# lh3/miniasm

Hardware: NVIDIA H100
Metric: paf_overlaps_per_sec_ingest_to_gfa (higher is better)
Workload: dtype int64/uint32 (+3 float32 predicates)

## Files before the change

### miniasm_b200/csrc/ingest_dev.cu

```cuda
#include "ingest_dev.cuh"
#include "shard_comm.cuh"
#include <cub/cub.cuh>

struct PLine {
	uint32_t ql, qs, qe, tl, ts, te, ml_rev, bl;
	uint32_t tdelta;
	uint32_t qnl, tnl;
	uint32_t nf;
};

struct __align__(16) PRec {
	uint32_t qs, qe, ts, te;
	uint32_t ml_rev;
	uint32_t bl_f;
	uint32_t slot_q, slot_t;
};
static_assert(sizeof(PRec) == 32, "PRec layout");
constexpr uint32_t NOSLOT = 0xffffffffu;

constexpr int NL_THREADS = 256;
constexpr int NL_PER_THREAD = 4;
constexpr uint64_t NL_TILE = (uint64_t)NL_THREADS * NL_PER_THREAD * 16;

__device__ __forceinline__ uint32_t nl_mask4(uint32_t w) { return __vcmpeq4(w, 0x0a0a0a0au); }
// ... 103 lines not shown
#ifdef __CUDA_ARCH__
				const int pos = off + __ffs(bits) - 1;
#else
				const int pos = off + __builtin_ctz(bits);
#endif
				bits &= bits - 1;
				if (pos >= 0 && pos < (int)len && nt < 11) tab[nt++ * 32] = (uint32_t)pos;
			}
		}
	}
	const uint32_t nf = nt + 1 < 11 ? nt + 1 : 11;
	#define COL_S(k) ((k) ? tab[((k) - 1) * 32] + 1 : 0u)
	#define COL_T(k) ((uint32_t)(k) < nt ? tab[(k) * 32] : len)
	memset(&r, 0, sizeof(r));
	r.nf = nf;
	r.qnl = COL_T(0);
	if (nf > 1) r.ql = num_field(p, COL_S(1), COL_T(1));
	if (nf > 2) r.qs = num_field(p, COL_S(2), COL_T(2));
	if (nf > 3) r.qe = num_field(p, COL_S(3), COL_T(3));
	if (nf > 4) { const uint32_t s4 = COL_S(4); r.ml_rev = (COL_T(4) > s4 && p[s4] == '-') ? 0x80000000u : 0; }
	if (nf > 5) {
		const uint32_t s5 = COL_S(5), t5 = COL_T(5);
		r.tnl = t5 - s5, r.tdelta = s5;
	}
	if (nf > 6) r.tl = num_field(p, COL_S(6), COL_T(6));
	if (nf > 7) r.ts = num_field(p, COL_S(7), COL_T(7));
	if (nf > 8) r.te = num_field(p, COL_S(8), COL_T(8));
	if (nf > 9) r.ml_rev |= num_field(p, COL_S(9), COL_T(9)) & 0x7fffffffu;
	if (nf > 10) r.bl = num_field(p, COL_S(10), COL_T(10));
	#undef COL_S
	#undef COL_T
}

struct NameTab {
	unsigned long long *key;
	unsigned long long *first;
	uint32_t *id;
	uint64_t mask;
	uint32_t *hits = nullptr;
};
constexpr int NT_OFF_BITS = 37;
constexpr unsigned long long NT_OFF_MASK = (1ull << NT_OFF_BITS) - 1;

__device__ __forceinline__ uint32_t tab_insert(const NameTab &t, const char *__restrict__ text, const char *nm, uint32_t nl, uint64_t goff, uint64_t occ,
                                               unsigned long long *overflow)
{
	const uint64_t h = name_hash(nm, 0, nl, 0);
	const unsigned long long mine = (h >> 37) << NT_OFF_BITS | (goff + 1);
	uint64_t s = h & t.mask;
	for (int probe = 0; probe < 1 << 14; ++probe, s = (s + 1) & t.mask) {
		unsigned long long k = t.key[s];
		if (k == 0) {
			k = atomicCAS(&t.key[s], 0ull, mine);
			if (k == 0) k = mine;
		}
		if ((k ^ mine) >> NT_OFF_BITS) continue;
		bool same = k == mine;
		if (!same) {
			const char *w = text + ((k & NT_OFF_MASK) - 1);
			same = true;
			for (uint32_t i = 0; same && i < nl; ++i) same = w[i] == nm[i];
			same = same && w[nl] == '\t';
		}
		if (!same) continue;
		if (t.first[s] > occ) atomicMin(&t.first[s], (unsigned long long)occ);
		return (uint32_t)s;
	}
	atomicAdd(overflow, 1ull);
	return 0;
}

constexpr int PT_THREADS = 128;
constexpr uint32_t PT_TILE = 8192;
constexpr uint32_t PT_OVER = 1024;
constexpr uint32_t PT_LIST = 1024;
static_assert(PT_TILE == PT_THREADS * 64, "each thread scans 64 bytes of its tile for line starts");
static_assert(PT_OVER % 16 == 0 && PT_OVER <= PT_TILE, "the overhang ends inside the tile after the parsed ones");

typedef cub::ScanTileState<unsigned long long> LineTileState;
typedef cub::TilePrefixCallbackOp<unsigned long long, ::cuda::std::plus<unsigned long long>, LineTileState> LinePrefixOp;

enum { PC_PARSED = 0, PC_STORED, PC_OVERFLOW, PC_LINES, PC_CUT, PC_N };

__device__ __forceinline__ uint32_t nl_bits_u4(const uint4 w)
{
	const uint32_t m[4] = { nl_mask4(w.x), nl_mask4(w.y), nl_mask4(w.z), nl_mask4(w.w) };
	uint32_t bits = 0;
	#pragma unroll
	for (int k = 0; k < 4; ++k) bits |= ((m[k] & 1) | (m[k] >> 7 & 2) | (m[k] >> 14 & 4) | (m[k] >> 21 & 8)) << (4 * k);
	return bits;
}

__global__ void k_tiles_init(LineTileState ts, int n_tile) { ts.InitializeStatus(n_tile); }

__global__ void __launch_bounds__(PT_THREADS)
k_parse_tiles(const char *__restrict__ text, size_t len, size_t avail, uint64_t t_lo, unsigned *tile_ctr, LineTileState tstate,
              int min_span, int min_match, int bi_dir, NameTab tab, PRec *out, uint64_t *start, uint64_t line_cap, unsigned long long *counts)
{
	typedef cub::BlockScan<uint32_t, PT_THREADS> BS;
	__shared__ __align__(16) char s_text[PT_TILE + PT_OVER + 16];
	__shared__ uint16_t s_start[PT_LIST + 1];
	__shared__ uint32_t s_vals[PT_THREADS / 32][11][32];
// ... 52 lines not shown
				if (e == ~0ull) atomicAdd(counts + PC_CUT, 1ull);
			}
		}
		__syncthreads();
		last_eol = s_eol;
	}
	unsigned n_parsed = 0, n_pass = 0;
	for (uint32_t r0 = 0; r0 < n; r0 += PT_LIST) {
		{
			uint32_t r = rank;
			uint64_t b = bits;
			if (line0) { if (r == r0) s_start[0] = 0; ++r; }
			for (; b && r <= r0 + PT_LIST; ++r, b &= b - 1)
				if (r >= r0) s_start[r - r0] = (uint16_t)(my0 + __ffsll((long long)b));
		}
		__syncthreads();
		const uint32_t cnt = n - r0 < PT_LIST ? n - r0 : PT_LIST;
		for (uint32_t j0 = 0; j0 < cnt; j0 += PT_THREADS) {
			const uint32_t j = j0 + threadIdx.x;
			const uint64_t i = first + r0 + j;
			uint32_t sq = NOSLOT, st = 0;
			if (j < cnt && i < line_cap) {
				const uint64_t s = b0 + s_start[j];
				uint64_t eol = r0 + j + 1 < n ? b0 + s_start[j + 1] - 1 : last_eol;
				if (eol != ~0ull) {
					const char *base = eol <= w_end ? s_text - b0 : text;
					if (eol - s > 1 && base[eol - 1] == '\r') --eol;
					PLine r;
					parse_line(base + s, base + eol, r, &s_vals[threadIdx.x >> 5][0][lane]);
					if (r.nf >= 10) {
						++n_parsed;
						if (!(r.qe - r.qs < (uint32_t)min_span || r.te - r.ts < (uint32_t)min_span || (int)(r.ml_rev & 0x7fffffffu) < min_match)) {
							++n_pass;
							sq = tab_insert(tab, text, base + s, r.qnl, s, 2 * i, counts + PC_OVERFLOW);
							st = tab_insert(tab, text, base + s + r.tdelta, r.tnl, s + r.tdelta, 2 * i + 1, counts + PC_OVERFLOW);
						}
					}
					start[i] = s;
					*reinterpret_cast<uint4*>(out + i) = make_uint4(r.qs, r.qe, r.ts, r.te);
					*(reinterpret_cast<uint4*>(out + i) + 1) = make_uint4(r.ml_rev, (r.bl & 0x7fffffffu) | (r.nf >= 11 ? 0x80000000u : 0u), sq, st);
				}
			}
			if (tab.hits) {
				const unsigned grp = __match_any_sync(0xffffffffu, sq);
				if (sq != NOSLOT && lane == (uint32_t)__ffs(grp) - 1) atomicAdd(&tab.hits[sq], (uint32_t)__popc(grp));
				if (sq != NOSLOT && bi_dir && st != sq) atomicAdd(&tab.hits[st], 1u);
			}
		}
		__syncthreads();
	}
	n_parsed = __reduce_add_sync(0xffffffffu, n_parsed), n_pass = __reduce_add_sync(0xffffffffu, n_pass);
	if (lane == 0) {
		if (n_parsed) atomicAdd(counts + PC_PARSED, (unsigned long long)n_parsed);
		if (n_pass) atomicAdd(counts + PC_STORED, (unsigned long long)n_pass);
	}
}

__device__ __forceinline__ uint32_t line_bl(const PRec *ln, uint64_t i, uint32_t carry_bl)
{
	if (ln[i].bl_f >> 31) return ln[i].bl_f & 0x7fffffffu;
	for (uint64_t j = i; j-- > 0;)
		if (ln[j].bl_f >> 31) return ln[j].bl_f & 0x7fffffffu;
	return carry_bl & 0x7fffffffu;
}

struct SlotUsed {
	const unsigned long long *first;
	__device__ __forceinline__ bool operator()(uint64_t s) const { return first[s] != ~0ull; }
};

__device__ __forceinline__ void occ_name(const char *text, const uint64_t *start, uint64_t occ, uint64_t *noff, uint32_t *nlen, uint32_t *slen)
{
	const char *p = text + start[occ >> 1];
	uint64_t q = 0;
	if (occ & 1) { int tabs = 0; while (tabs < 5) tabs += p[q++] == '\t'; }
	uint64_t e = q;
	while (p[e] != '\t') ++e;
	*noff = start[occ >> 1] + q, *nlen = (uint32_t)(e - q);
	uint64_t f = e + 1;
	while (p[f] != '\t') ++f;
	*slen = field_to_u32(p + e + 1, p + f);
}

__global__ void k_nocont_mark(const PRec *ln, uint64_t n_lines, const char *text, const uint64_t *start, int max_hang, float int_frac, uint8_t *excl)
{
	for (uint64_t i = blockIdx.x * (uint64_t)blockDim.x + threadIdx.x; i < n_lines; i += (uint64_t)gridDim.x * blockDim.x) {
		const PRec r = ln[i];
		if (r.slot_q == NOSLOT) continue;
		uint64_t no; uint32_t nl, ql, tl;
		occ_name(text, start, 2 * i, &no, &nl, &ql);
		occ_name(text, start, 2 * i + 1, &no, &nl, &tl);
		const bool rev = r.ml_rev >> 31;
		const int l5 = (int)(rev ? tl - r.te : r.ts), l3 = (int)(rev ? r.ts : tl - r.te);
		if (ql >> 1 > tl) {
			if (l5 > max_hang >> 2 || l3 > max_hang >> 2 || (float)(r.te - r.ts) < __fmul_rn((float)tl, int_frac)) continue;
			if ((int)r.qs - l5 > max_hang << 1 && (int)(ql - r.qe) - l3 > max_hang << 1) excl[r.slot_t] = 1;
		} else if (ql < tl >> 1) {
			if (r.qs > (uint32_t)(max_hang >> 2) || ql - r.qe > (uint32_t)(max_hang >> 2) || (float)(r.qe - r.qs) < __fmul_rn((float)ql, int_frac)) continue;
			if (l5 - (int)r.qs > max_hang << 1 && l3 - (int)(ql - r.qe) > max_hang << 1) excl[r.slot_q] = 1;
		}
	}
}

__global__ void k_nocont_drop(PRec *ln, uint64_t n_lines, const uint8_t *excl, int bi_dir, NameTab t)
{
	for (uint64_t i = blockIdx.x * (uint64_t)blockDim.x + threadIdx.x; i < n_lines; i += (uint64_t)gridDim.x * blockDim.x) {
		const uint32_t sq = ln[i].slot_q, st = ln[i].slot_t;
		if (sq == NOSLOT) continue;
		if (excl[sq] || excl[st]) { ln[i].slot_q = NOSLOT; continue; }
		if (t.first[sq] > 2 * i) atomicMin(&t.first[sq], (unsigned long long)(2 * i));
		if (t.first[st] > 2 * i + 1) atomicMin(&t.first[st], (unsigned long long)(2 * i + 1));
		atomicAdd(&t.hits[sq], 1u);
		if (bi_dir && st != sq) atomicAdd(&t.hits[st], 1u);
	}
}

__global__ void k_count_u8(const uint8_t *a, uint64_t n, unsigned long long *out)
{
	unsigned c = 0;
	for (uint64_t i = blockIdx.x * (uint64_t)blockDim.x + threadIdx.x; i < n; i += (uint64_t)gridDim.x * blockDim.x) c += a[i] != 0;
	c = __reduce_add_sync(0xffffffffu, c);
	if ((threadIdx.x & 31) == 0 && c) atomicAdd(out, (unsigned long long)c);
}

__global__ void k_dict_pairs(const uint64_t *slots, uint32_t n, NameTab t, unsigned long long *first_out)
{
	for (uint32_t i = blockIdx.x * blockDim.x + threadIdx.x; i < n; i += gridDim.x * blockDim.x) first_out[i] = t.first[slots[i]];
}

__global__ void k_dict_rank(const unsigned long long *first_sorted, const uint64_t *slot_sorted, uint32_t n, NameTab t,
                            const char *text, const uint64_t *start, uint64_t *noff, uint32_t *nlen, uint32_t *slen, unsigned long long *tot_len,
                            uint32_t *read_cnt)
{
	unsigned long long sum = 0;
	for (uint32_t i = blockIdx.x * blockDim.x + threadIdx.x; i < n; i += gridDim.x * blockDim.x) {
		t.id[slot_sorted[i]] = i;
		read_cnt[i] = t.hits[slot_sorted[i]];
		occ_name(text, start, first_sorted[i], &noff[i], &nlen[i], &slen[i]);
		sum += slen[i];
	}
	typedef cub::BlockReduce<unsigned long long, 256> BR;
	__shared__ typename BR::TempStorage ts;
	unsigned long long s = BR(ts).Sum(sum);
	if (threadIdx.x == 0 && s) atomicAdd(tot_len, s);
}

__global__ void k_hit_emit(const PRec *ln, uint64_t n_lines, int bi_dir, NameTab t, const uint32_t *__restrict__ first, uint32_t *cur, DHit *out)
{
	for (uint64_t i = blockIdx.x * (uint64_t)blockDim.x + threadIdx.x; i < n_lines; i += (uint64_t)gridDim.x * blockDim.x) {
		const PRec r = ln[i];
		if (r.slot_q == NOSLOT) continue;
		const uint32_t qid = t.id[r.slot_q], tid = t.id[r.slot_t], bl = line_bl(ln, i, 0), ord = (uint32_t)(2 * i);
		uint4 *o = reinterpret_cast<uint4*>(out + first[qid] + atomicAdd(&cur[qid], 1u));
		o[0] = make_uint4(r.qs, ord, r.qe, tid);
		o[1] = make_uint4(r.ts, r.te, r.ml_rev, bl);
		if (bi_dir && qid != tid) {
			o = reinterpret_cast<uint4*>(out + first[tid] + atomicAdd(&cur[tid], 1u));
			o[0] = make_uint4(r.ts, ord + 1, r.te, qid);
			o[1] = make_uint4(r.qs, r.qe, r.ml_rev, bl);
		}
// ... 1 lines not shown
}

uint64_t *dev_line_starts(MabDev &d, const char *d_text, size_t len, uint64_t *n_lines_out)
{
	const uint64_t n_tile = (len + NL_TILE - 1) / NL_TILE;
	uint64_t *cnt = mab_alloc<uint64_t>(d, n_tile + 1);
	uint64_t *base = mab_alloc<uint64_t>(d, n_tile + 1);
	MAB_LAUNCH(d, k_nl_count, mab_grid(n_tile, 1, MAB_SMS * 32u), NL_THREADS, 0, d_text, len, n_tile, cnt);
	size_t tb = 0;
	cub::DeviceScan::ExclusiveSum(nullptr, tb, cnt, base, (int64_t)(n_tile + 1), d.stream);
	void *tmp = d.tmp(tb);
	cub::DeviceScan::ExclusiveSum(tmp, tb, cnt, base, (int64_t)(n_tile + 1), d.stream);
	++d.n_lib;
	uint64_t n_nl;
	MAB_CUDA(cudaMemcpyAsync(&n_nl, base + n_tile, 8, cudaMemcpyDeviceToHost, d.stream));
	d.sync();
	const uint64_t n_lines = n_nl + 1;
	uint64_t *start = mab_alloc<uint64_t>(d, n_lines + 1);
	MAB_CUDA(cudaMemsetAsync(start, 0, 8, d.stream));
	MAB_LAUNCH(d, k_nl_write, mab_grid(n_tile, 1, MAB_SMS * 32u), NL_THREADS, 0, d_text, len, n_tile, base, start + 1);
	d.free(cnt); d.free(base);
	*n_lines_out = n_lines;
	return start;
}

void names_free(MabDev &d, DNames &n)
{
	d.free(n.off); d.free(n.nlen); d.free(n.slen);
	n = DNames();
}

static inline uint32_t bits_for(uint64_t x) { uint32_t b = 0; while (x) ++b, x >>= 1; return b ? b : 1; }

static NameTab tab_alloc(MabDev &d, uint64_t cap, bool with_hits)
{
	NameTab tab;
	tab.key = (unsigned long long*)mab_alloc<uint64_t>(d, cap);
	tab.first = (unsigned long long*)mab_alloc<uint64_t>(d, cap);
	tab.id = mab_alloc<uint32_t>(d, cap);
	tab.mask = cap - 1;
	MAB_CUDA(cudaMemsetAsync(tab.key, 0, cap * 8, d.stream));
	MAB_CUDA(cudaMemsetAsync(tab.first, 0xff, cap * 8, d.stream));
	if (with_hits) {
		tab.hits = mab_alloc<uint32_t>(d, cap);
		MAB_CUDA(cudaMemsetAsync(tab.hits, 0, cap * 4, d.stream));
	}
	return tab;
}

static void tab_free(MabDev &d, NameTab &t)
{
	d.free(t.key); d.free(t.first); d.free(t.id);
	if (t.hits) d.free(t.hits);
	t = NameTab{nullptr, nullptr, nullptr, 0};
}

struct Parsed {
	uint64_t *start = nullptr;
	PRec *ln = nullptr;
	NameTab tab{nullptr, nullptr, nullptr, 0};
	uint64_t cap = 0, n_lines = 0, n_parsed = 0;
};

static inline uint64_t line_estimate(size_t len) { return len / 24 + 1024; }
static inline uint64_t tab_cap_for(uint64_t line_cap) { uint64_t cap = 1ull << 20; while (cap < line_cap / 8) cap <<= 1; return cap; }

static LineTileState tiles_alloc(MabDev &d, uint64_t n_tile, void **mem)
{
	if (n_tile >= (1ull << 31) - 64) { fprintf(stderr, "[E::miniasm_b200] more than 2^31 tiles of PAF on one GPU\n"); exit(73); }
	size_t bytes = 0;
	MAB_CUDA(LineTileState::AllocationSize((int)n_tile, bytes));
	*mem = d.alloc(bytes);
	LineTileState ts;
	MAB_CUDA(ts.Init((int)n_tile, *mem, bytes));
	return ts;
}

static void tiles_reset(MabDev &d, LineTileState ts, uint64_t n_tile)
{
	MAB_LAUNCH(d, k_tiles_init, mab_grid(n_tile, 256, 1u << 30), 256, 0, ts, (int)n_tile);
}

static void parse_resident(MabDev &d, const char *d_text, size_t len, int min_span, int min_match, int bi_dir, bool count_hits, Parsed &p)
{
	const uint64_t n_tile = (len + PT_TILE - 1) / PT_TILE;
	uint64_t line_cap = line_estimate(len), cap = tab_cap_for(line_cap);
	unsigned *ctr = mab_alloc<unsigned>(d, 1);
	void *ts_mem = nullptr;
	const LineTileState ts = tiles_alloc(d, n_tile, &ts_mem);
	for (;;) {
		p.start = mab_alloc<uint64_t>(d, line_cap);
		p.ln = mab_alloc<PRec>(d, line_cap);
		p.tab = tab_alloc(d, cap, count_hits);
// ... 83 lines not shown
	p.cap = cap;
	return true;
}

void ingest_paf_stream(MabDev &d, char *d_text, const char *host_text, size_t len, int min_span, int min_match, int bi_dir,
                       DHits &h, DNames &names, IngestStats &st)
{
	memset(&st, 0, sizeof(st));
	names = DNames();
	h.n = 0, h.n_seq = 0;
	if (len == 0) { dh_reserve(d, h, 1); return; }
	if (len >= (1ull << NT_OFF_BITS) - 1) { fprintf(stderr, "[E::miniasm_b200] more than 2^37 bytes of PAF on one GPU\n"); exit(73); }
	Parsed p;
	if (!stream_parse(d, d_text, host_text, len, min_span, min_match, bi_dir, true, p)) {
		ingest_paf(d, d_text, len, min_span, min_match, bi_dir, h, names, st, nullptr);
		return;
	}
	st.n_parsed = p.n_parsed, st.n_lines = p.n_lines;
	d.trace("ingest:stream (copy + parse + dictionary + hit counts)");
	ingest_finish(d, d_text, len, p.start, p.ln, p.n_lines, p.tab, p.cap, bi_dir, nullptr, h, names, st);
}

static void ingest_finish(MabDev &d, const char *d_text, size_t len, uint64_t *start, PRec *ln, uint64_t n_lines, NameTab tab, uint64_t cap, int bi_dir,
                          const NoContParams *nocont, DHits &h, DNames &names, IngestStats &st)
{
	if (2 * n_lines >= (1ull << 32)) { fprintf(stderr, "[E::miniasm_b200] more than 2^31 PAF lines on one GPU\n"); exit(73); }
	d.trace("ingest:dictionary");
	if (nocont) {
		uint8_t *excl = mab_alloc<uint8_t>(d, cap);
		MAB_CUDA(cudaMemsetAsync(excl, 0, cap, d.stream));
		MAB_LAUNCH(d, k_nocont_mark, mab_grid(n_lines, 256), 256, 0, ln, n_lines, d_text, start, nocont->max_hang, nocont->int_frac, excl);
		d.zero_scal(SC_AUX, 1);
		MAB_LAUNCH(d, k_count_u8, mab_grid(cap, 256), 256, 0, excl, cap, d.d_scal + SC_AUX);
		MAB_CUDA(cudaMemsetAsync(tab.first, 0xff, cap * 8, d.stream));
		MAB_CUDA(cudaMemsetAsync(tab.hits, 0, cap * 4, d.stream));
		MAB_LAUNCH(d, k_nocont_drop, mab_grid(n_lines, 256), 256, 0, ln, n_lines, excl, bi_dir, tab);
		st.n_dropped = d.get_scal(SC_AUX);
		d.free(excl);
		d.trace("ingest:-R prefilter");
	}
	uint64_t *slots = mab_alloc<uint64_t>(d, cap);
	uint32_t n_seq;
	{
		cub::CountingInputIterator<uint64_t> pos(0);
		SlotUsed used{tab.first};
		size_t tb = 0;
		unsigned long long *d_n = d.d_scal + SC_NSEL;
		cub::DeviceSelect::If(nullptr, tb, pos, slots, d_n, (int64_t)cap, used, d.stream);
		void *tmp = d.tmp(tb);
		cub::DeviceSelect::If(tmp, tb, pos, slots, d_n, (int64_t)cap, used, d.stream);
		++d.n_lib;
		uint64_t n = d.get_scal(SC_NSEL);
		if (n >= (1ull << 31)) { fprintf(stderr, "[E::miniasm_b200] more than 2^31 reads\n"); exit(73); }
		n_seq = (uint32_t)n;
	}
	names.n_seq = n_seq;
	names.off = mab_alloc<uint64_t>(d, n_seq); names.nlen = mab_alloc<uint32_t>(d, n_seq); names.slen = mab_alloc<uint32_t>(d, n_seq);
	uint32_t *read_cnt = mab_alloc<uint32_t>(d, (size_t)n_seq + 1), *first = mab_alloc<uint32_t>(d, (size_t)n_seq + 1);
	MAB_CUDA(cudaMemsetAsync(read_cnt + n_seq, 0, 4, d.stream));
	if (n_seq) {
		unsigned long long *fa = (unsigned long long*)mab_alloc<uint64_t>(d, n_seq), *fb = (unsigned long long*)mab_alloc<uint64_t>(d, n_seq);
		uint64_t *sb = mab_alloc<uint64_t>(d, n_seq);
		MAB_LAUNCH(d, k_dict_pairs, mab_grid(n_seq, 256), 256, 0, slots, n_seq, tab, fa);
		cub::DoubleBuffer<unsigned long long> dk(fa, fb);
		cub::DoubleBuffer<uint64_t> dv(slots, sb);
		size_t tb = 0;
		int end_bit = (int)bits_for(2 * n_lines + 1);
		cub::DeviceRadixSort::SortPairs(nullptr, tb, dk, dv, (int)n_seq, 0, end_bit, d.stream);
		void *tmp = d.tmp(tb);
		cub::DeviceRadixSort::SortPairs(tmp, tb, dk, dv, (int)n_seq, 0, end_bit, d.stream);
		++d.n_lib;
		d.zero_scal(SC_AUX, 1);
		MAB_LAUNCH(d, k_dict_rank, mab_grid(n_seq, 256), 256, 0, dk.Current(), dv.Current(), n_seq, tab, d_text, start, names.off, names.nlen, names.slen, d.d_scal + SC_AUX,
		           read_cnt);
		st.tot_len = d.get_scal(SC_AUX);
		d.free(fa); d.free(fb); d.free(sb);
	}
	d.free(slots);
// ... 15 lines not shown
	dh_sort_buckets(d, h, first);
	d.free(read_cnt); d.free(first);
	d.trace("ingest:sort_hits");
}

extern "C" int mab_test_parse_line(const char *line, size_t len, uint32_t *out)
{
	static uint32_t vals[11 * 32];
	PLine r;
	size_t eol = len;
	if (eol > 1 && line[eol - 1] == '\r') --eol;
	parse_line(line, line + eol, r, vals);
	out[0] = r.nf, out[1] = r.ql, out[2] = r.qs, out[3] = r.qe, out[4] = r.ml_rev >> 31, out[5] = r.tl, out[6] = r.ts, out[7] = r.te;
	out[8] = r.ml_rev & 0x7fffffffu, out[9] = r.bl, out[10] = r.qnl, out[11] = r.tnl, out[12] = r.tdelta;
	return 0;
}

__global__ void k_last_bl(const PRec *ln, uint64_t n_lines, unsigned long long *out)
{
	unsigned long long mx = 0;
	for (uint64_t i = blockIdx.x * (uint64_t)blockDim.x + threadIdx.x; i < n_lines; i += (uint64_t)gridDim.x * blockDim.x)
		if (ln[i].bl_f >> 31) mx = i + 1;
	#pragma unroll
	for (int o = 16; o; o >>= 1) { unsigned long long t = __shfl_xor_sync(0xffffffffu, mx, o); mx = t > mx ? t : mx; }
	if ((threadIdx.x & 31) == 0 && mx) atomicMax(out, mx);
}

struct GEntry { unsigned long long hash, first; uint32_t slen, nlen; };

__global__ void k_local_entries(const uint64_t *slots, uint32_t n, NameTab t, const char *text, const uint64_t *start, uint64_t line_base, uint64_t seed,
                                GEntry *ent, uint32_t *name_sz, uint64_t *name_off)
{
	for (uint32_t i = blockIdx.x * blockDim.x + threadIdx.x; i < n; i += gridDim.x * blockDim.x) {
		const uint64_t occ = t.first[slots[i]];
		GEntry e;
		uint64_t no;
		occ_name(text, start, occ, &no, &e.nlen, &e.slen);
		e.hash = name_hash(text + no, 0, e.nlen, seed), e.first = 2 * line_base + occ;
		ent[i] = e;
		name_sz[i] = e.nlen, name_off[i] = no;
	}
}

__global__ void k_local_names(uint32_t n, const uint64_t *name_off, const uint32_t *name_sz, const char *text, const uint64_t *pos, char *out)
{
	for (uint32_t i = blockIdx.x * blockDim.x + threadIdx.x; i < n; i += gridDim.x * blockDim.x) {
		const char *src = text + name_off[i];
		char *dst = out + pos[i];
		for (uint32_t k = 0; k < name_sz[i]; ++k) dst[k] = src[k];
	}
}

struct U32ToU64i { __host__ __device__ __forceinline__ uint64_t operator()(uint32_t x) const { return x; } };

struct GTab { unsigned long long *key, *first; uint32_t *win, *id; uint64_t mask; };

__global__ void k_gtab_insert(const GEntry *ent, uint64_t n, GTab t, uint32_t *slot_of, unsigned long long *overflow)
{
	for (uint64_t i = blockIdx.x * (uint64_t)blockDim.x + threadIdx.x; i < n; i += (uint64_t)gridDim.x * blockDim.x) {
		const unsigned long long h = ent[i].hash;
		uint64_t s = h & t.mask;
		uint32_t found = 0xffffffffu;
		for (int probe = 0; probe < 1 << 14; ++probe, s = (s + 1) & t.mask) {
			unsigned long long k = t.key[s];
			if (k == 0) { k = atomicCAS(&t.key[s], 0ull, h); if (k == 0) k = h; }
			if (k == h) { atomicMin(&t.first[s], ent[i].first); found = (uint32_t)s; break; }
		}
// ... 191 lines not shown
	h.n = 0, h.n_seq = 0;
	const int G = sc.world;
	if (len >= (1ull << NT_OFF_BITS) - 1) { fprintf(stderr, "[E::miniasm_b200] more than 2^37 bytes of PAF on one GPU\n"); exit(73); }
	Parsed p;
	bool have = false;
	if (host_text && len) {
		have = stream_parse(d, d_text, host_text, len, min_span, min_match, bi_dir, false, p);
		d.trace("shard-ingest:stream (copy + parse + dictionary)");
	}
	if (!have) parse_resident(d, d_text, len, min_span, min_match, bi_dir, false, p);
	uint64_t *start = p.start, n_lines = p.n_lines, cap = p.cap, n_parsed = p.n_parsed;
	PRec *ln = p.ln;
	NameTab tab = p.tab;
	st.n_parsed = n_parsed;
	std::vector<uint64_t> all_lines = sc_allgather_u64(d, sc, n_lines);
	uint64_t line_base = 0, n_lines_all = 0;
	for (int r = 0; r < G; ++r) { if (r < sc.rank) line_base += all_lines[r]; n_lines_all += all_lines[r]; }
	st.n_lines = n_lines_all;
	d.trace("shard-ingest:parse+filter+local dictionary");
	uint32_t carry = 0;
	{
		d.zero_scal(SC_TMP0, 1);
		if (n_lines) MAB_LAUNCH(d, k_last_bl, mab_grid(n_lines, 256), 256, 0, ln, n_lines, d.d_scal + SC_TMP0);
		uint64_t last11 = d.get_scal(SC_TMP0);
		uint32_t my_bl = 0;
		if (last11) { MAB_CUDA(cudaMemcpyAsync(&my_bl, &ln[last11 - 1].bl_f, 4, cudaMemcpyDeviceToHost, d.stream)); d.sync(); my_bl &= 0x7fffffffu; }
		std::vector<uint64_t> bls = sc_allgather_u64(d, sc, last11 ? ((uint64_t)1 << 32 | my_bl) : 0);
		for (int r = 0; r < sc.rank; ++r) if (bls[r] >> 32) carry = (uint32_t)bls[r];
	}
	uint32_t n_ent = 0;
	uint64_t *slots = mab_alloc<uint64_t>(d, cap);
	{
		cub::CountingInputIterator<uint64_t> pos(0);
		SlotUsed used{tab.first};
		size_t tb = 0;
		unsigned long long *d_n = d.d_scal + SC_NSEL;
		cub::DeviceSelect::If(nullptr, tb, pos, slots, d_n, (int64_t)cap, used, d.stream);
		void *tmp = d.tmp(tb);
		cub::DeviceSelect::If(tmp, tb, pos, slots, d_n, (int64_t)cap, used, d.stream);
		++d.n_lib;
		n_ent = (uint32_t)d.get_scal(SC_NSEL);
	}
	GTab gt{nullptr, nullptr, nullptr, nullptr, 0};
	GEntry *g_ent = nullptr;
	char *g_names = nullptr;
	uint64_t *g_pos = nullptr;
	uint32_t *slot_of = nullptr;
	uint64_t n_ent_all = 0, name_bytes_all = 0, my_ent_off = 0;
	uint64_t seed = 0;
	for (int attempt = 0;; ++attempt) {
		GEntry *ent = mab_alloc<GEntry>(d, n_ent);
		uint32_t *nsz = mab_alloc<uint32_t>(d, (size_t)n_ent + 1);
		uint64_t *npos = mab_alloc<uint64_t>(d, (size_t)n_ent + 1), *nsrc = mab_alloc<uint64_t>(d, (size_t)n_ent + 1);
		uint64_t my_name_bytes = 0;
		char *my_names = nullptr;
		if (n_ent) {
			MAB_LAUNCH(d, k_local_entries, mab_grid(n_ent, 256), 256, 0, slots, n_ent, tab, d_text, start, line_base, seed, ent, nsz, nsrc);
			size_t tb = 0;
			cub::DeviceScan::ExclusiveSum(nullptr, tb, nsz, npos, (int)n_ent, d.stream);
			void *tmp = d.tmp(tb);
			cub::DeviceScan::ExclusiveSum(tmp, tb, nsz, npos, (int)n_ent, d.stream);
			++d.n_lib;
			uint64_t lp; uint32_t ls;
			MAB_CUDA(cudaMemcpyAsync(&lp, npos + n_ent - 1, 8, cudaMemcpyDeviceToHost, d.stream));
			MAB_CUDA(cudaMemcpyAsync(&ls, nsz + n_ent - 1, 4, cudaMemcpyDeviceToHost, d.stream));
			d.sync();
			my_name_bytes = lp + ls;
// ... 186 lines not shown
	std::vector<uint64_t> hits_all = sc_allgather_u64(d, sc, n_recv), parsed_all = sc_allgather_u64(d, sc, st.n_parsed);
	st.n_hits = st.n_parsed = 0;
	for (int r = 0; r < G; ++r) st.n_hits += hits_all[r], st.n_parsed += parsed_all[r];
	st.n_seq = n_seq;
	dh_sort(d, h);
	d.trace("shard-ingest:sort");
}

enum { WS_PARSED = 0, WS_STORED, WS_TAB_FULL, WS_STORE_FULL, WS_STORE_USED, WS_BAD, WS_EMITTED,
       WS_LINE_IN, WS_BL_IN,
       WS_LINE_OUT, WS_BL_OUT,
       WS_N };

struct WinTab {
	NameTab t;
	char *store;
	uint64_t store_cap;
};

template <bool CG>
__device__ __forceinline__ bool name_at(const char *w, const char *nm, uint32_t nl)
{
	for (uint32_t i = 0; i < nl; ++i) if ((CG ? __ldcg(w + i) : w[i]) != nm[i]) return false;
	return (CG ? __ldcg(w + nl) : w[nl]) == '\t';
}

__device__ __forceinline__ uint32_t win_insert(const WinTab &t, const char *win, const char *nm, uint32_t nl, uint64_t woff, uint64_t occ, uint32_t slen,
                                               unsigned long long *ws)
{
	const uint64_t h = name_hash(nm, 0, nl, 0);
	const unsigned long long frag = (h >> 37) << NT_OFF_BITS, mine = frag | (t.store_cap + woff + 1);
	uint64_t s = h & t.t.mask;
	for (int probe = 0; probe < 1 << 14; ++probe, s = (s + 1) & t.t.mask) {
		unsigned long long k = t.t.key[s];
		bool fresh = false;
		if (k == 0) {
			k = atomicCAS(&t.t.key[s], 0ull, mine);
			if (k == 0) k = mine, fresh = true;
		}
		if ((k ^ mine) >> NT_OFF_BITS) continue;
		if (fresh) {
			const unsigned long long at = atomicAdd(ws + WS_STORE_USED, (unsigned long long)nl + 1);
			if (at + nl + 1 <= t.store_cap) {
				for (uint32_t i = 0; i < nl; ++i) t.store[at + i] = nm[i];
				t.store[at + nl] = '\t';
				__threadfence();
				atomicExch(&t.t.key[s], frag | (at + 1));
			} else atomicAdd(ws + WS_STORE_FULL, 1ull);
		} else {
			const uint64_t off = (k & NT_OFF_MASK) - 1;
			if (!name_at<true>(off < t.store_cap ? t.store + off : win + (off - t.store_cap), nm, nl)) continue;
		}
		const unsigned long long v = occ << 32 | slen;
		if (t.t.first[s] > v) atomicMin(&t.t.first[s], v);
		return (uint32_t)s;
	}
	atomicAdd(ws + WS_TAB_FULL, 1ull);
	return 0;
}

__device__ __forceinline__ uint32_t win_find(const WinTab &t, const char *nm, uint32_t nl)
{
	const uint64_t h = name_hash(nm, 0, nl, 0);
	uint64_t s = h & t.t.mask;
	for (int probe = 0; probe < 1 << 14; ++probe, s = (s + 1) & t.t.mask) {
		const unsigned long long k = t.t.key[s];
		if (k == 0) break;
		if ((k >> NT_OFF_BITS) == (h >> 37) && name_at<false>(t.store + ((k & NT_OFF_MASK) - 1), nm, nl)) return (uint32_t)s;
	}
	return NOSLOT;
}

__device__ uint32_t win_prev_bl(const char *text, uint64_t s, unsigned long long carry)
{
	while (s > 0) {
		uint64_t eol = s - 1, p = eol;
		while (p > 0 && text[p - 1] != '\n') --p;
		if (eol - p > 1 && text[eol - 1] == '\r') --eol;
		uint64_t q = p;
		int tabs = 0;
		for (; q < eol && tabs < 10; ++q) tabs += text[q] == '\t';
		if (tabs == 10) {
			uint64_t f = q;
			while (f < eol && text[f] != '\t') ++f;
			return num_field(text + q, 0, (uint32_t)(f - q)) & 0x7fffffffu;
		}
		s = p;
	}
	return (uint32_t)carry & 0x7fffffffu;
}

template <int PASS>
__global__ void __launch_bounds__(PT_THREADS)
k_win_tiles(const char *__restrict__ text, size_t len, unsigned *tile_ctr, LineTileState tstate, int min_span, int min_match, int bi_dir, WinTab tab,
            const uint32_t *__restrict__ bfirst, uint32_t *cur, DHit *out, unsigned long long *ws)
{
	typedef cub::BlockScan<uint32_t, PT_THREADS> BS;
	__shared__ __align__(16) char s_text[PT_TILE + PT_OVER + 16];
	__shared__ uint16_t s_start[PT_LIST + 1];
// ... 108 lines not shown
							}
						}
					}
				}
			}
			if (PASS == 1) {
				const unsigned grp = __match_any_sync(0xffffffffu, sq);
				if (sq != NOSLOT && lane == (uint32_t)__ffs(grp) - 1) atomicAdd(&tab.t.hits[sq], (uint32_t)__popc(grp));
				if (sq != NOSLOT && bi_dir && st != sq) atomicAdd(&tab.t.hits[st], 1u);
			}
		}
		__syncthreads();
	}
	n_parsed = __reduce_add_sync(0xffffffffu, n_parsed), n_pass = __reduce_add_sync(0xffffffffu, n_pass);
	if (PASS == 2) {
		n_bad = __reduce_add_sync(0xffffffffu, n_bad), n_emit = __reduce_add_sync(0xffffffffu, n_emit);
		#pragma unroll
		for (int o = 16; o; o >>= 1) { const unsigned long long y = __shfl_xor_sync(0xffffffffu, last11, o); last11 = y > last11 ? y : last11; }
	}
	if (lane == 0) {
		if (n_parsed) atomicAdd(ws + WS_PARSED, (unsigned long long)n_parsed);
		if (n_pass) atomicAdd(ws + WS_STORED, (unsigned long long)n_pass);
		if (n_bad) atomicAdd(ws + WS_BAD, (unsigned long long)n_bad);
		if (n_emit) atomicAdd(ws + WS_EMITTED, (unsigned long long)n_emit);
		if (last11) atomicMax(ws + WS_BL_OUT, last11);
	}
}

__global__ void k_win_rank(const unsigned long long *first_sorted, const uint64_t *slot_sorted, uint32_t n, WinTab t, uint64_t *noff, uint32_t *nlen, uint32_t *slen,
                           unsigned long long *tot_len, uint32_t *read_cnt)
{
	unsigned long long sum = 0;
	for (uint32_t i = blockIdx.x * blockDim.x + threadIdx.x; i < n; i += gridDim.x * blockDim.x) {
		const uint64_t s = slot_sorted[i], off = (t.t.key[s] & NT_OFF_MASK) - 1;
		t.t.id[s] = i;
		read_cnt[i] = t.t.hits[s];
		uint32_t l = 0;
		while (t.store[off + l] != '\t') ++l;
		noff[i] = off, nlen[i] = l, slen[i] = (uint32_t)first_sorted[i];
		sum += slen[i];
	}
	typedef cub::BlockReduce<unsigned long long, 256> BR;
	__shared__ typename BR::TempStorage ts;
	unsigned long long s = BR(ts).Sum(sum);
	if (threadIdx.x == 0 && s) atomicAdd(tot_len, s);
}

struct WinRun {
	MabDev &d;
	const TextSource &src;
	size_t cap;
	char *host[2] = {nullptr, nullptr}, *dev[2] = {nullptr, nullptr};
	cudaEvent_t copied[2], parsed[2];
	void *ts_mem = nullptr;
	LineTileState ts;
	unsigned *ctr = nullptr;
	unsigned long long *ws = nullptr;

	WinRun(MabDev &dev_, const TextSource &s, size_t w) : d(dev_), src(s), cap(0)
	{
		for (int i = 0; i < 2; ++i) {
			MAB_CUDA(cudaEventCreateWithFlags(&copied[i], cudaEventDisableTiming));
			MAB_CUDA(cudaEventCreateWithFlags(&parsed[i], cudaEventDisableTiming));
		}
		ctr = mab_alloc<unsigned>(d, 1);
		ws = (unsigned long long*)mab_alloc<uint64_t>(d, WS_N);
		if (!d.copy_stream) MAB_CUDA(cudaStreamCreateWithFlags(&d.copy_stream, cudaStreamNonBlocking));
// ... 87 lines not shown
	d.trace("ingest:begin");
	if (window_bytes < (64u << 10)) window_bytes = 64u << 10;
	WinRun w(d, src, (window_bytes + PT_TILE - 1) / PT_TILE * PT_TILE);
	uint64_t cap = tab_cap_for(line_estimate(size_hint)), store_cap = size_hint / 32 > (8u << 20) ? size_hint / 32 : (8u << 20);
	unsigned long long ws[WS_N];
	uint64_t n_bytes = 0;
	WinTab tab;
	for (;;) {
		tab.t = tab_alloc(d, cap, true);
		tab.store = (char*)d.alloc(store_cap), tab.store_cap = store_cap;
		const bool ok = win_pass<1>(w, min_span, min_match, bi_dir, tab, nullptr, nullptr, nullptr, &n_bytes);
		if (ok) { MAB_CUDA(cudaMemcpyAsync(ws, w.ws, sizeof(ws), cudaMemcpyDeviceToHost, d.stream)); d.sync(); }
		if (ok && !ws[WS_TAB_FULL] && !ws[WS_STORE_FULL]) break;
		tab_free(d, tab.t); d.free(tab.store);
		if (!ok) return false;
		if (ws[WS_TAB_FULL]) cap <<= 2;
		if (ws[WS_STORE_FULL]) store_cap <<= 2;
		if (cap > (1ull << 32)) { fprintf(stderr, "[E::miniasm_b200] read-name table overflow\n"); exit(77); }
	}
	const uint64_t n_lines = ws[WS_LINE_IN];
	st.n_lines = n_lines, st.n_parsed = ws[WS_PARSED];
	const uint64_t n_stored = ws[WS_STORED];
	if (2 * n_lines >= (1ull << 32)) { fprintf(stderr, "[E::miniasm_b200] more than 2^31 PAF lines on one GPU\n"); exit(73); }
	d.trace("ingest:windowed pass 1 (parse + dictionary + hit counts)");
	if (n_bytes == 0) {
		tab_free(d, tab.t); d.free(tab.store);
		dh_reserve(d, h, 1);
		return true;
	}
	uint64_t *slots = mab_alloc<uint64_t>(d, cap);
	uint32_t n_seq;
	{
		cub::CountingInputIterator<uint64_t> pos(0);
		SlotUsed used{tab.t.first};
		size_t tb = 0;
		unsigned long long *d_n = d.d_scal + SC_NSEL;
		cub::DeviceSelect::If(nullptr, tb, pos, slots, d_n, (int64_t)cap, used, d.stream);
		void *tmp = d.tmp(tb);
		cub::DeviceSelect::If(tmp, tb, pos, slots, d_n, (int64_t)cap, used, d.stream);
		++d.n_lib;
		const uint64_t n = d.get_scal(SC_NSEL);
		if (n >= (1ull << 31)) { fprintf(stderr, "[E::miniasm_b200] more than 2^31 reads\n"); exit(73); }
		n_seq = (uint32_t)n;
	}
	names.n_seq = n_seq;
	names.off = mab_alloc<uint64_t>(d, n_seq); names.nlen = mab_alloc<uint32_t>(d, n_seq); names.slen = mab_alloc<uint32_t>(d, n_seq);
	uint32_t *read_cnt = mab_alloc<uint32_t>(d, (size_t)n_seq + 1), *first = mab_alloc<uint32_t>(d, (size_t)n_seq + 1);
	MAB_CUDA(cudaMemsetAsync(read_cnt + n_seq, 0, 4, d.stream));
	if (n_seq) {
		unsigned long long *fa = (unsigned long long*)mab_alloc<uint64_t>(d, n_seq), *fb = (unsigned long long*)mab_alloc<uint64_t>(d, n_seq);
		uint64_t *sb = mab_alloc<uint64_t>(d, n_seq);
		MAB_LAUNCH(d, k_dict_pairs, mab_grid(n_seq, 256), 256, 0, slots, n_seq, tab.t, fa);
		cub::DoubleBuffer<unsigned long long> dk(fa, fb);
		cub::DoubleBuffer<uint64_t> dv(slots, sb);
		size_t tb = 0;
		cub::DeviceRadixSort::SortPairs(nullptr, tb, dk, dv, (int)n_seq, 32, 64, d.stream);
		void *tmp = d.tmp(tb);
		cub::DeviceRadixSort::SortPairs(tmp, tb, dk, dv, (int)n_seq, 32, 64, d.stream);
		++d.n_lib;
		d.zero_scal(SC_AUX, 1);
		MAB_LAUNCH(d, k_win_rank, mab_grid(n_seq, 256), 256, 0, dk.Current(), dv.Current(), n_seq, tab, names.off, names.nlen, names.slen, d.d_scal + SC_AUX, read_cnt);
		st.tot_len = d.get_scal(SC_AUX);
		d.free(fa); d.free(fb); d.free(sb);
	}
	d.free(slots);
	d.trace("ingest:rank_ids");
	dh_bucket_first(d, read_cnt, n_seq, first);
// ... 31 lines not shown
```

Before: 1.630 billion.

## Interleave name-table key/first into 16-byte slots and batch query/target probes

The name hash table's separate key and first arrays become one array of 16-byte slots, so a single vector load fetches both and a probe touches one cache line. Query and target name inserts are split into begin/probe/witness/settle phases so both first-slot loads and the witness-name loads are in flight together, with a fast path for a hit on the first probe with names up to 7 bytes. Name comparison now uses 8-byte word loads instead of a byte loop. Table reset becomes a custom kernel instead of two memsets, which adds kernel launches and relies on unaligned-to-aligned word reads near the end of the text buffer.

```diff
diff --git a/miniasm_b200/csrc/ingest_dev.cu b/miniasm_b200/csrc/ingest_dev.cu
--- a/miniasm_b200/csrc/ingest_dev.cu
+++ b/miniasm_b200/csrc/ingest_dev.cu
@@ -159,9 +159,13 @@
 	#undef COL_T
 }
 
+struct __align__(16) NSlot {
+	unsigned long long key;
+	unsigned long long first;
+};
+static_assert(sizeof(NSlot) == 16, "NSlot layout");
 struct NameTab {
-	unsigned long long *key;
-	unsigned long long *first;
+	NSlot *slot;
 	uint32_t *id;
 	uint64_t mask;
 	uint32_t *hits = nullptr;
@@ -169,32 +173,82 @@
 constexpr int NT_OFF_BITS = 37;
 constexpr unsigned long long NT_OFF_MASK = (1ull << NT_OFF_BITS) - 1;
 
-__device__ __forceinline__ uint32_t tab_insert(const NameTab &t, const char *__restrict__ text, const char *nm, uint32_t nl, uint64_t goff, uint64_t occ,
-                                               unsigned long long *overflow)
+__device__ __forceinline__ ulonglong2 slot_load(const NameTab &t, uint64_t s) { return *reinterpret_cast<const ulonglong2*>(t.slot + s); }
+
+__device__ __forceinline__ uint64_t ld_bytes(const char *p, uint32_t m)
+{
+	const uintptr_t a = (uintptr_t)p & ~(uintptr_t)7;
+	const uint32_t o = (uint32_t)((uintptr_t)p & 7);
+	uint64_t w = *reinterpret_cast<const uint64_t*>(a) >> (8 * o);
+	if (o + m > 8) w |= *reinterpret_cast<const uint64_t*>(a + 8) << (64 - 8 * o);
+	return m == 8 ? w : w & ((1ull << (8 * m)) - 1);
+}
+
+__device__ __forceinline__ bool bytes_eq(const char *a, const char *b, uint32_t n)
+{
+	for (uint32_t i = 0; i < n; i += 8) {
+		const uint32_t m = n - i < 8 ? n - i : 8;
+		if (ld_bytes(a + i, m) != ld_bytes(b + i, m)) return false;
+	}
+	return true;
+}
+
+struct NameIns {
+	const char *nm;
+	unsigned long long mine;
+	unsigned long long occ;
+	uint64_t s;
+	uint32_t nl;
+	ulonglong2 v;
+	uint64_t w0;
+};
+
+__device__ __forceinline__ void name_begin(NameIns &n, const NameTab &t, const char *nm, uint32_t nl, uint64_t goff, uint64_t occ)
 {
 	const uint64_t h = name_hash(nm, 0, nl, 0);
-	const unsigned long long mine = (h >> 37) << NT_OFF_BITS | (goff + 1);
-	uint64_t s = h & t.mask;
-	for (int probe = 0; probe < 1 << 14; ++probe, s = (s + 1) & t.mask) {
-		unsigned long long k = t.key[s];
+	n.nm = nm, n.nl = nl, n.occ = occ;
+	n.mine = (h >> 37) << NT_OFF_BITS | (goff + 1);
+	n.s = h & t.mask;
+}
+
+__device__ __forceinline__ bool frag_witness(unsigned long long k, unsigned long long mine) { return k != 0 && k != mine && !((k ^ mine) >> NT_OFF_BITS); }
+
+__device__ __forceinline__ void name_probe(NameIns &n, const NameTab &t) { n.v = slot_load(t, n.s); }
+
+__device__ __forceinline__ void name_witness(NameIns &n, const char *__restrict__ text)
+{
+	n.w0 = frag_witness(n.v.x, n.mine) ? ld_bytes(text + ((n.v.x & NT_OFF_MASK) - 1), n.nl + 1 < 8 ? n.nl + 1 : 8) : 0;
+}
+
+__device__ __forceinline__ uint32_t name_settle_slow(NameIns n, const NameTab &t, const char *__restrict__ text, unsigned long long *overflow)
+{
+	const uint32_t m0 = n.nl + 1 < 8 ? n.nl + 1 : 8;
+	for (int probe = 0; probe < 1 << 14; ++probe, n.s = (n.s + 1) & t.mask) {
+		const ulonglong2 v = slot_load(t, n.s);
+		unsigned long long k = v.x;
 		if (k == 0) {
-			k = atomicCAS(&t.key[s], 0ull, mine);
-			if (k == 0) k = mine;
-		}
-		if ((k ^ mine) >> NT_OFF_BITS) continue;
-		bool same = k == mine;
-		if (!same) {
+			k = atomicCAS(&t.slot[n.s].key, 0ull, n.mine);
+			if (k == 0) k = n.mine;
+		}
+		if ((k ^ n.mine) >> NT_OFF_BITS) continue;
+		if (k != n.mine) {
 			const char *w = text + ((k & NT_OFF_MASK) - 1);
-			same = true;
-			for (uint32_t i = 0; same && i < nl; ++i) same = w[i] == nm[i];
-			same = same && w[nl] == '\t';
-		}
-		if (!same) continue;
-		if (t.first[s] > occ) atomicMin(&t.first[s], (unsigned long long)occ);
-		return (uint32_t)s;
+			if (ld_bytes(w, m0) != ld_bytes(n.nm, m0) || (n.nl + 1 > 8 && !bytes_eq(w + 8, n.nm + 8, n.nl - 7))) continue;
+		}
+		if (v.y > n.occ) atomicMin(&t.slot[n.s].first, n.occ);
+		return (uint32_t)n.s;
 	}
 	atomicAdd(overflow, 1ull);
 	return 0;
+}
+
+__device__ __forceinline__ uint32_t name_settle(const NameIns &n, const NameTab &t, const char *__restrict__ text, unsigned long long *overflow)
+{
+	if (n.v.x == n.mine || (frag_witness(n.v.x, n.mine) && n.nl + 1 <= 8 && n.w0 == ld_bytes(n.nm, n.nl + 1))) {
+		if (n.v.y > n.occ) atomicMin(&t.slot[n.s].first, n.occ);
+		return (uint32_t)n.s;
+	}
+	return name_settle_slow(n, t, text, overflow);
 }
 
 constexpr int PT_THREADS = 128;
@@ -313,8 +367,13 @@
 						++n_parsed;
 						if (!(r.qe - r.qs < (uint32_t)min_span || r.te - r.ts < (uint32_t)min_span || (int)(r.ml_rev & 0x7fffffffu) < min_match)) {
 							++n_pass;
-							sq = tab_insert(tab, text, base + s, r.qnl, s, 2 * i, counts + PC_OVERFLOW);
-							st = tab_insert(tab, text, base + s + r.tdelta, r.tnl, s + r.tdelta, 2 * i + 1, counts + PC_OVERFLOW);
+							NameIns nq, nt;
+							name_begin(nq, tab, base + s, r.qnl, s, 2 * i);
+							name_begin(nt, tab, base + s + r.tdelta, r.tnl, s + r.tdelta, 2 * i + 1);
+							name_probe(nq, tab), name_probe(nt, tab);
+							name_witness(nq, text), name_witness(nt, text);
+							sq = name_settle(nq, tab, text, counts + PC_OVERFLOW);
+							st = name_settle(nt, tab, text, counts + PC_OVERFLOW);
 						}
 					}
 					start[i] = s;
@@ -346,8 +405,8 @@
 }
 
 struct SlotUsed {
-	const unsigned long long *first;
-	__device__ __forceinline__ bool operator()(uint64_t s) const { return first[s] != ~0ull; }
+	const NSlot *slot;
+	__device__ __forceinline__ bool operator()(uint64_t s) const { return slot[s].first != ~0ull; }
 };
 
 __device__ __forceinline__ void occ_name(const char *text, const uint64_t *start, uint64_t occ, uint64_t *noff, uint32_t *nlen, uint32_t *slen)
@@ -389,8 +448,8 @@
 		const uint32_t sq = ln[i].slot_q, st = ln[i].slot_t;
 		if (sq == NOSLOT) continue;
 		if (excl[sq] || excl[st]) { ln[i].slot_q = NOSLOT; continue; }
-		if (t.first[sq] > 2 * i) atomicMin(&t.first[sq], (unsigned long long)(2 * i));
-		if (t.first[st] > 2 * i + 1) atomicMin(&t.first[st], (unsigned long long)(2 * i + 1));
+		if (t.slot[sq].first > 2 * i) atomicMin(&t.slot[sq].first, (unsigned long long)(2 * i));
+		if (t.slot[st].first > 2 * i + 1) atomicMin(&t.slot[st].first, (unsigned long long)(2 * i + 1));
 		atomicAdd(&t.hits[sq], 1u);
 		if (bi_dir && st != sq) atomicAdd(&t.hits[st], 1u);
 	}
@@ -406,7 +465,7 @@
 
 __global__ void k_dict_pairs(const uint64_t *slots, uint32_t n, NameTab t, unsigned long long *first_out)
 {
-	for (uint32_t i = blockIdx.x * blockDim.x + threadIdx.x; i < n; i += gridDim.x * blockDim.x) first_out[i] = t.first[slots[i]];
+	for (uint32_t i = blockIdx.x * blockDim.x + threadIdx.x; i < n; i += gridDim.x * blockDim.x) first_out[i] = t.slot[slots[i]].first;
 }
 
 __global__ void k_dict_rank(const unsigned long long *first_sorted, const uint64_t *slot_sorted, uint32_t n, NameTab t,
@@ -474,15 +533,21 @@
 
 static inline uint32_t bits_for(uint64_t x) { uint32_t b = 0; while (x) ++b, x >>= 1; return b ? b : 1; }
 
+__global__ void k_tab_reset(NSlot *slot, uint64_t cap, bool keys)
+{
+	for (uint64_t s = blockIdx.x * (uint64_t)blockDim.x + threadIdx.x; s < cap; s += (uint64_t)gridDim.x * blockDim.x) {
+		if (keys) *reinterpret_cast<ulonglong2*>(slot + s) = make_ulonglong2(0ull, ~0ull);
+		else slot[s].first = ~0ull;
+	}
+}
+
 static NameTab tab_alloc(MabDev &d, uint64_t cap, bool with_hits)
 {
 	NameTab tab;
-	tab.key = (unsigned long long*)mab_alloc<uint64_t>(d, cap);
-	tab.first = (unsigned long long*)mab_alloc<uint64_t>(d, cap);
+	tab.slot = reinterpret_cast<NSlot*>(mab_alloc<ulonglong2>(d, cap));
 	tab.id = mab_alloc<uint32_t>(d, cap);
 	tab.mask = cap - 1;
-	MAB_CUDA(cudaMemsetAsync(tab.key, 0, cap * 8, d.stream));
-	MAB_CUDA(cudaMemsetAsync(tab.first, 0xff, cap * 8, d.stream));
+	MAB_LAUNCH(d, k_tab_reset, mab_grid(cap, 256), 256, 0, tab.slot, cap, true);
 	if (with_hits) {
 		tab.hits = mab_alloc<uint32_t>(d, cap);
 		MAB_CUDA(cudaMemsetAsync(tab.hits, 0, cap * 4, d.stream));
@@ -492,15 +557,15 @@
 
 static void tab_free(MabDev &d, NameTab &t)
 {
-	d.free(t.key); d.free(t.first); d.free(t.id);
+	d.free(t.slot); d.free(t.id);
 	if (t.hits) d.free(t.hits);
-	t = NameTab{nullptr, nullptr, nullptr, 0};
+	t = NameTab{nullptr, nullptr, 0};
 }
 
 struct Parsed {
 	uint64_t *start = nullptr;
 	PRec *ln = nullptr;
-	NameTab tab{nullptr, nullptr, nullptr, 0};
+	NameTab tab{nullptr, nullptr, 0};
 	uint64_t cap = 0, n_lines = 0, n_parsed = 0;
 };
 
@@ -650,7 +715,7 @@
 		MAB_LAUNCH(d, k_nocont_mark, mab_grid(n_lines, 256), 256, 0, ln, n_lines, d_text, start, nocont->max_hang, nocont->int_frac, excl);
 		d.zero_scal(SC_AUX, 1);
 		MAB_LAUNCH(d, k_count_u8, mab_grid(cap, 256), 256, 0, excl, cap, d.d_scal + SC_AUX);
-		MAB_CUDA(cudaMemsetAsync(tab.first, 0xff, cap * 8, d.stream));
+		MAB_LAUNCH(d, k_tab_reset, mab_grid(cap, 256), 256, 0, tab.slot, cap, false);
 		MAB_CUDA(cudaMemsetAsync(tab.hits, 0, cap * 4, d.stream));
 		MAB_LAUNCH(d, k_nocont_drop, mab_grid(n_lines, 256), 256, 0, ln, n_lines, excl, bi_dir, tab);
 		st.n_dropped = d.get_scal(SC_AUX);
@@ -661,7 +726,7 @@
 	uint32_t n_seq;
 	{
 		cub::CountingInputIterator<uint64_t> pos(0);
-		SlotUsed used{tab.first};
+		SlotUsed used{tab.slot};
 		size_t tb = 0;
 		unsigned long long *d_n = d.d_scal + SC_NSEL;
 		cub::DeviceSelect::If(nullptr, tb, pos, slots, d_n, (int64_t)cap, used, d.stream);
@@ -743,7 +808,7 @@
                                 GEntry *ent, uint32_t *name_sz, uint64_t *name_off)
 {
 	for (uint32_t i = blockIdx.x * blockDim.x + threadIdx.x; i < n; i += gridDim.x * blockDim.x) {
-		const uint64_t occ = t.first[slots[i]];
+		const uint64_t occ = t.slot[slots[i]].first;
 		GEntry e;
 		uint64_t no;
 		occ_name(text, start, occ, &no, &e.nlen, &e.slen);
@@ -1001,7 +1066,7 @@
 	uint64_t *slots = mab_alloc<uint64_t>(d, cap);
 	{
 		cub::CountingInputIterator<uint64_t> pos(0);
-		SlotUsed used{tab.first};
+		SlotUsed used{tab.slot};
 		size_t tb = 0;
 		unsigned long long *d_n = d.d_scal + SC_NSEL;
 		cub::DeviceSelect::If(nullptr, tb, pos, slots, d_n, (int64_t)cap, used, d.stream);
@@ -1254,10 +1319,10 @@
 	const unsigned long long frag = (h >> 37) << NT_OFF_BITS, mine = frag | (t.store_cap + woff + 1);
 	uint64_t s = h & t.t.mask;
 	for (int probe = 0; probe < 1 << 14; ++probe, s = (s + 1) & t.t.mask) {
-		unsigned long long k = t.t.key[s];
+		unsigned long long k = t.t.slot[s].key;
 		bool fresh = false;
 		if (k == 0) {
-			k = atomicCAS(&t.t.key[s], 0ull, mine);
+			k = atomicCAS(&t.t.slot[s].key, 0ull, mine);
 			if (k == 0) k = mine, fresh = true;
 		}
 		if ((k ^ mine) >> NT_OFF_BITS) continue;
@@ -1267,14 +1332,14 @@
 				for (uint32_t i = 0; i < nl; ++i) t.store[at + i] = nm[i];
 				t.store[at + nl] = '\t';
 				__threadfence();
-				atomicExch(&t.t.key[s], frag | (at + 1));
+				atomicExch(&t.t.slot[s].key, frag | (at + 1));
 			} else atomicAdd(ws + WS_STORE_FULL, 1ull);
 		} else {
 			const uint64_t off = (k & NT_OFF_MASK) - 1;
 			if (!name_at<true>(off < t.store_cap ? t.store + off : win + (off - t.store_cap), nm, nl)) continue;
 		}
 		const unsigned long long v = occ << 32 | slen;
-		if (t.t.first[s] > v) atomicMin(&t.t.first[s], v);
+		if (t.t.slot[s].first > v) atomicMin(&t.t.slot[s].first, v);
 		return (uint32_t)s;
 	}
 	atomicAdd(ws + WS_TAB_FULL, 1ull);
@@ -1286,7 +1351,7 @@
 	const uint64_t h = name_hash(nm, 0, nl, 0);
 	uint64_t s = h & t.t.mask;
 	for (int probe = 0; probe < 1 << 14; ++probe, s = (s + 1) & t.t.mask) {
-		const unsigned long long k = t.t.key[s];
+		const unsigned long long k = t.t.slot[s].key;
 		if (k == 0) break;
 		if ((k >> NT_OFF_BITS) == (h >> 37) && name_at<false>(t.store + ((k & NT_OFF_MASK) - 1), nm, nl)) return (uint32_t)s;
 	}
@@ -1461,7 +1526,7 @@
 {
 	unsigned long long sum = 0;
 	for (uint32_t i = blockIdx.x * blockDim.x + threadIdx.x; i < n; i += gridDim.x * blockDim.x) {
-		const uint64_t s = slot_sorted[i], off = (t.t.key[s] & NT_OFF_MASK) - 1;
+		const uint64_t s = slot_sorted[i], off = (t.t.slot[s].key & NT_OFF_MASK) - 1;
 		t.t.id[s] = i;
 		read_cnt[i] = t.t.hits[s];
 		uint32_t l = 0;
@@ -1615,7 +1680,7 @@
 	uint32_t n_seq;
 	{
 		cub::CountingInputIterator<uint64_t> pos(0);
-		SlotUsed used{tab.t.first};
+		SlotUsed used{tab.t.slot};
 		size_t tb = 0;
 		unsigned long long *d_n = d.d_scal + SC_NSEL;
 		cub::DeviceSelect::If(nullptr, tb, pos, slots, d_n, (int64_t)cap, used, d.stream);
```

Result: no change. 1.631 billion (median of 6 runs) (+0.1%).
